# alipay/PainlessInferenceAcceleration

Hardware: NVIDIA H100
Metric: accepted tokens/sec @ Llama-2-7B 64-draft/8-branch; mean accepted len/step (higher is better)
Workload: dtype bf16

## Files before the change

painlessinferenceacceleration_b200/csrc/gemm_ws.cu:

```cuda
#include <cuda.h>
#include <cuda_bf16.h>

#include <new>

#include "common.cuh"

namespace pia {
namespace gemm {

constexpr int BMW = 128;
constexpr int BK = 64;
constexpr int TOK = 64;
constexpr int NTHREADS = 288;
constexpr int PRODUCER_WARP = 8;
constexpr int W_BYTES = BMW * BK * 2, X_BYTES = TOK * BK * 2, STAGE_BYTES = W_BYTES + X_BYTES;
constexpr int XCH_BYTES = TOK * 64 * 2;
constexpr int smem_total(int nstage) { return nstage * STAGE_BYTES + 256 + XCH_BYTES + 1024; }
constexpr int ACC_OFF = 32 * 1024, ACC_LD = TOK + 4;
static_assert(ACC_OFF + BMW * ACC_LD * 4 <= 4 * STAGE_BYTES, "accumulator staging must fit in the pipeline stages");

__device__ __forceinline__ uint32_t smem_u32(const void *p) { return (uint32_t)__cvta_generic_to_shared(p); }
__device__ __forceinline__ void mbar_init(uint32_t bar, int count) {
  asm volatile("mbarrier.init.shared::cta.b64 [%0], %1;" ::"r"(bar), "r"(count));
}
__device__ __forceinline__ void mbar_arrive(uint32_t bar) {
  asm volatile("mbarrier.arrive.shared::cta.b64 _, [%0];" ::"r"(bar) : "memory");
}
__device__ __forceinline__ void mbar_expect_tx(uint32_t bar, uint32_t bytes) {
  asm volatile("mbarrier.arrive.expect_tx.shared::cta.b64 _, [%0], %1;" ::"r"(bar), "r"(bytes) : "memory");
}
__device__ __forceinline__ void mbar_wait(uint32_t bar, uint32_t parity) {
  uint32_t done;
  do {
    asm volatile(
        "{\n\t.reg .pred p;\n\t"
        "mbarrier.try_wait.parity.shared::cta.b64 p, [%1], %2;\n\t"
        "selp.u32 %0, 1, 0, p;\n\t}"
        : "=r"(done)
        : "r"(bar), "r"(parity)
        : "memory");
  } while (!done);
}
__device__ __forceinline__ void cluster_sync_all() {
  asm volatile("barrier.cluster.arrive.release.aligned;\n\tbarrier.cluster.wait.acquire.aligned;" ::: "memory");
}
__device__ __forceinline__ uint32_t map_to_cta(uint32_t local_smem_addr, uint32_t cta_rank) {
  uint32_t r;
  asm volatile("mapa.shared::cluster.u32 %0, %1, %2;" : "=r"(r) : "r"(local_smem_addr), "r"(cta_rank));
  return r;
}
__device__ __forceinline__ void st_cluster_f4(uint32_t addr, float a, float b, float c, float d) {
  asm volatile("st.shared::cluster.v4.f32 [%0], {%1, %2, %3, %4};" ::"r"(addr), "f"(a), "f"(b), "f"(c), "f"(d) : "memory");
}
__device__ __forceinline__ void tma_load_2d(uint32_t dst, const CUtensorMap *map, uint32_t bar, int c0, int c1) {
  asm volatile(
      "cp.async.bulk.tensor.2d.shared::cluster.global.mbarrier::complete_tx::bytes [%0], [%1, {%3, %4}], [%2];"
      ::"r"(dst), "l"(map), "r"(bar), "r"(c0), "r"(c1)
      : "memory");
}
__device__ __forceinline__ void tma_load_3d(uint32_t dst, const CUtensorMap *map, uint32_t bar, int c0, int c1, int c2) {
  asm volatile(
      "cp.async.bulk.tensor.3d.shared::cluster.global.mbarrier::complete_tx::bytes [%0], [%1, {%3, %4, %5}], [%2];"
      ::"r"(dst), "l"(map), "r"(bar), "r"(c0), "r"(c1), "r"(c2)
      : "memory");
}
__device__ __forceinline__ uint64_t kmajor_desc(uint32_t saddr) {
  uint64_t d = 0;
  d |= (uint64_t)((saddr >> 4) & 0x3FFF);
  d |= (uint64_t)1 << 16;
  d |= (uint64_t)(1024 >> 4) << 32;
  d |= (uint64_t)1 << 62;
  return d;
}
__device__ __forceinline__ void wgmma_fence() { asm volatile("wgmma.fence.sync.aligned;" ::: "memory"); }
__device__ __forceinline__ void wgmma_commit() { asm volatile("wgmma.commit_group.sync.aligned;" ::: "memory"); }
__device__ __forceinline__ void wgmma_wait_all() { asm volatile("wgmma.wait_group.sync.aligned 0;" ::: "memory"); }
__device__ __forceinline__ void fence_acc(float (&d)[32]) {
#pragma unroll
  for (int i = 0; i < 32; ++i) asm volatile("" : "+f"(d[i])::"memory");
}
__device__ __forceinline__ void wgmma_m64n64k16(float (&d)[32], uint64_t desc_a, uint64_t desc_b) {
  asm volatile(
      "{\n\t"
      "wgmma.mma_async.sync.aligned.m64n64k16.f32.bf16.bf16 "
      "{%0, %1, %2, %3, %4, %5, %6, %7, %8, %9, %10, %11, %12, %13, %14, %15, "
      "%16, %17, %18, %19, %20, %21, %22, %23, %24, %25, %26, %27, %28, %29, %30, %31}, %32, %33, 1, 1, 1, 0, 0;\n\t}"
      : "+f"(d[0]), "+f"(d[1]), "+f"(d[2]), "+f"(d[3]), "+f"(d[4]), "+f"(d[5]), "+f"(d[6]), "+f"(d[7]), "+f"(d[8]),
        "+f"(d[9]), "+f"(d[10]), "+f"(d[11]), "+f"(d[12]), "+f"(d[13]), "+f"(d[14]), "+f"(d[15]), "+f"(d[16]),
        "+f"(d[17]), "+f"(d[18]), "+f"(d[19]), "+f"(d[20]), "+f"(d[21]), "+f"(d[22]), "+f"(d[23]), "+f"(d[24]),
        "+f"(d[25]), "+f"(d[26]), "+f"(d[27]), "+f"(d[28]), "+f"(d[29]), "+f"(d[30]), "+f"(d[31])
      : "l"(desc_a), "l"(desc_b)
      : "memory");
}
__device__ __forceinline__ void mma_stage(float (&acc)[32], uint32_t wa, uint32_t xa) {
  wgmma_fence();
#pragma unroll
  for (int j = 0; j < BK / 16; ++j) wgmma_m64n64k16(acc, kmajor_desc(wa + j * 32), kmajor_desc(xa + j * 32));
  wgmma_commit();
  wgmma_wait_all();
  fence_acc(acc);
}
__device__ __forceinline__ int frag_row(int warp, int lane, int h) { return 16 * (warp & 3) + (lane >> 2) + 8 * h; }
__device__ __forceinline__ int frag_tok(int lane, int i) { return 8 * i + 2 * (lane & 3); }

struct Params {
  int N, K, n_split, chunks_per_split, n_chunks, rows, tiled;
  int groups, w_group_rows, x_group_chunks;
  long long out_group_stride;
  int cluster;
  int silu;
  int no_pdl;
  __nv_bfloat16 *out_bf16;
  float *out_f32;
};

template <int NSTAGE>
__global__ void __launch_bounds__(NTHREADS, NSTAGE <= 4 ? 2 : 1)
k_gemm_ws(const __grid_constant__ CUtensorMap map_w, const __grid_constant__ CUtensorMap map_x, Params p) {
  constexpr int SMEM_BAR = NSTAGE * STAGE_BYTES;
  extern __shared__ uint8_t smem_raw[];
  const uint32_t base = (smem_u32(smem_raw) + 1023u) & ~1023u;
  uint8_t *sm = smem_raw + (base - smem_u32(smem_raw));
  const int tid = threadIdx.x, warp = tid >> 5, lane = tid & 31;
  const uint32_t bar_full = base + SMEM_BAR, bar_empty = bar_full + 8 * NSTAGE;
  const int tile = p.cluster ? blockIdx.y : blockIdx.x, split = p.cluster ? blockIdx.x : blockIdx.y;
  const int n0 = tile * BMW;
  const int grp = blockIdx.z;
  const int xk0 = grp * p.x_group_chunks;
  const int c0 = split * p.chunks_per_split;
  int c1 = c0 + p.chunks_per_split;
  if (c1 > p.n_chunks) c1 = p.n_chunks;
  const int nch = c1 - c0;

  if (tid == 0) {
    for (int s = 0; s < NSTAGE; ++s) { mbar_init(bar_full + 8 * s, 1); mbar_init(bar_empty + 8 * s, 8); }
    asm volatile("fence.mbarrier_init.release.cluster;" ::: "memory");
  }
  __syncwarp();
  if (!p.no_pdl) pdl_launch_dependents();
  __syncthreads();

  if (warp == PRODUCER_WARP) {
    if (lane == 0) {
      auto load_w = [&](int i, int s) {
        const uint32_t wd = base + s * STAGE_BYTES;
        if (p.tiled) tma_load_3d(wd, &map_w, bar_full + 8 * s, 0, 0, tile * p.n_chunks + c0 + i);
        else tma_load_2d(wd, &map_w, bar_full + 8 * s, (c0 + i) * BK, grp * p.w_group_rows + n0);
      };
      const int pre = nch < NSTAGE ? nch : NSTAGE;
      for (int i = 0; i < pre; ++i) {
        mbar_expect_tx(bar_full + 8 * i, STAGE_BYTES);
        load_w(i, i);
      }
      pdl_wait();
      for (int i = 0; i < pre; ++i) tma_load_2d(base + i * STAGE_BYTES + W_BYTES, &map_x, bar_full + 8 * i, (xk0 + c0 + i) * BK, 0);
      for (int i = pre; i < nch; ++i) {
        const int s = i % NSTAGE, ph = (i / NSTAGE) & 1;
        mbar_wait(bar_empty + 8 * s, ph ^ 1);
        mbar_expect_tx(bar_full + 8 * s, STAGE_BYTES);
        load_w(i, s);
        tma_load_2d(base + s * STAGE_BYTES + W_BYTES, &map_x, bar_full + 8 * s, (xk0 + c0 + i) * BK, 0);
      }
    }
    __syncwarp();
    if (p.cluster) { cluster_sync_all(); cluster_sync_all(); }
    return;
  }

  pdl_wait();
  const int wg = warp >> 2;
  float acc[32];
#pragma unroll
  for (int j = 0; j < 32; ++j) acc[j] = 0.f;
  for (int i = 0; i < nch; ++i) {
    const int s = i % NSTAGE, ph = (i / NSTAGE) & 1;
    mbar_wait(bar_full + 8 * s, ph);
    const uint32_t wa = base + s * STAGE_BYTES, xa = wa + W_BYTES;
    mma_stage(acc, wa + wg * 64 * 128, xa);
    __syncwarp();
    if (lane == 0) mbar_arrive(bar_empty + 8 * s);
  }
  float *accs = reinterpret_cast<float *>(sm + ACC_OFF);
  asm volatile("bar.sync 2, 256;" ::: "memory");
#pragma unroll
  for (int h = 0; h < 2; ++h) {
    const int r = wg * 64 + frag_row(warp, lane, h);
#pragma unroll
    for (int i = 0; i < 8; ++i)
      *reinterpret_cast<float2 *>(accs + r * ACC_LD + frag_tok(lane, i)) = make_float2(acc[4 * i + 2 * h], acc[4 * i + 2 * h + 1]);
  }
  asm volatile("bar.sync 2, 256;" ::: "memory");
  if (wg == 1) {
    if (p.cluster) { cluster_sync_all(); cluster_sync_all(); }
    return;
  }

  const int q = warp;
  const int n = n0 + q * 32 + lane;
  uint32_t v[64];
  {
    const float4 *src = reinterpret_cast<const float4 *>(accs + (q * 32 + lane) * ACC_LD);
#pragma unroll
    for (int t = 0; t < 16; ++t) {
      const float4 a = src[t];
      v[4 * t] = __float_as_uint(a.x); v[4 * t + 1] = __float_as_uint(a.y);
      v[4 * t + 2] = __float_as_uint(a.z); v[4 * t + 3] = __float_as_uint(a.w);
    }
  }
  if (p.cluster) {
    const int cs = p.cluster, RS = BMW / cs;
    cluster_sync_all();
    {
      const int row = q * 32 + lane;
      const int owner = row / RS, rl = row % RS;
      const uint32_t dst = map_to_cta(base + (uint32_t)((split * 16) * RS + rl) * 16, owner);
#pragma unroll
      for (int tq = 0; tq < 16; ++tq)
        st_cluster_f4(dst + (uint32_t)(tq * RS) * 16, __uint_as_float(v[4 * tq]), __uint_as_float(v[4 * tq + 1]),
                      __uint_as_float(v[4 * tq + 2]), __uint_as_float(v[4 * tq + 3]));
    }
    cluster_sync_all();
    {
      const int e = warp * 32 + lane;
      const int rl = e % RS, tg = e / RS;
      const int qpt = RS / 8;
      const int n_out = n0 + split * RS + rl;
      const float4 *buf = reinterpret_cast<const float4 *>(sm);
      __nv_bfloat16 *ob = p.out_bf16 + grp * p.out_group_stride;
      if (n_out < p.N) {
        for (int tq = tg * qpt; tq < (tg + 1) * qpt; ++tq) {
          float4 a = buf[(0 * 16 + tq) * RS + rl];
          for (int src = 1; src < cs; ++src) {
            const float4 b = buf[(src * 16 + tq) * RS + rl];
            a.x += b.x; a.y += b.y; a.z += b.z; a.w += b.w;
          }
          const int t0 = 4 * tq;
          if (t0 < p.rows) ob[(long long)t0 * p.N + n_out] = __float2bfloat16_rn(a.x);
          if (t0 + 1 < p.rows) ob[(long long)(t0 + 1) * p.N + n_out] = __float2bfloat16_rn(a.y);
          if (t0 + 2 < p.rows) ob[(long long)(t0 + 2) * p.N + n_out] = __float2bfloat16_rn(a.z);
          if (t0 + 3 < p.rows) ob[(long long)(t0 + 3) * p.N + n_out] = __float2bfloat16_rn(a.w);
        }
      }
    }
  } else
  if (p.silu) {
    __nv_bfloat16 *xu = reinterpret_cast<__nv_bfloat16 *>(sm + SMEM_BAR + 256);
    __nv_bfloat16 *xg = xu + 32 * 64;
    const int rr = (q & 1) * 32 + lane;
    if (q >= 2) {
#pragma unroll
      for (int t = 0; t < 32; ++t) xu[t * 64 + rr] = __float2bfloat16_rn(__uint_as_float(v[t]));
    } else {
#pragma unroll
      for (int t = 0; t < 32; ++t) xg[t * 64 + rr] = __float2bfloat16_rn(__uint_as_float(v[32 + t]));
    }
    asm volatile("bar.sync 1, 128;" ::: "memory");
    const int col = tile * 64 + rr;
    const int inter = p.N >> 1;
    if (col < inter) {
      const int tb = q < 2 ? 0 : 32;
#pragma unroll
      for (int t = 0; t < 32; ++t) {
        if (tb + t < p.rows) {
          const float g = q < 2 ? __bfloat162float(__float2bfloat16_rn(__uint_as_float(v[t]))) : __bfloat162float(xg[t * 64 + rr]);
          const float u = q < 2 ? __bfloat162float(xu[t * 64 + rr]) : __bfloat162float(__float2bfloat16_rn(__uint_as_float(v[32 + t])));
          const float sg = __bfloat162float(__float2bfloat16_rn(g / (1.f + expf(-g))));
          p.out_bf16[(long long)(tb + t) * inter + col] = __float2bfloat16_rn(sg * u);
        }
      }
    }
  } else
  if (n < p.N) {
    if (p.n_split == 1) {
#pragma unroll
      for (int t = 0; t < TOK; ++t)
        if (t < p.rows) p.out_bf16[grp * p.out_group_stride + (long long)t * p.N + n] = __float2bfloat16_rn(__uint_as_float(v[t]));
    } else {
      float *o = p.out_f32 + (long long)split * TOK * p.N;
#pragma unroll
      for (int t = 0; t < TOK; ++t)
        if (t < p.rows) o[(long long)t * p.N + n] = __uint_as_float(v[t]);
    }
  }
}


struct SkParams {
  int N, n_tiles, n_chunks, rows, max_contrib;
  long long units;
  __nv_bfloat16 *out;
  float *ws;
  int *flags;
};

__device__ __forceinline__ long long sk_begin(long long b, long long U, int G) { return b * U / G; }
__device__ __forceinline__ int sk_cta_of(long long x, long long U, int G) {
  int b = (int)(x * G / U);
  while (b + 1 < G && sk_begin(b + 1, U, G) <= x) ++b;
  while (b > 0 && sk_begin(b, U, G) > x) --b;
  return b;
}

constexpr int SK_STAGES = 8;
constexpr int SK_SMEM_BAR = SK_STAGES * STAGE_BYTES;
constexpr int SK_SMEM_TOTAL = SK_SMEM_BAR + 256 + 1024;

__global__ void __launch_bounds__(NTHREADS, 1)
k_gemm_sk(const __grid_constant__ CUtensorMap map_w, const __grid_constant__ CUtensorMap map_x, SkParams p) {
  extern __shared__ uint8_t smem_raw[];
  const uint32_t base = (smem_u32(smem_raw) + 1023u) & ~1023u;
  const int tid = threadIdx.x, warp = tid >> 5, lane = tid & 31;
  const uint32_t bar_full = base + SK_SMEM_BAR, bar_empty = bar_full + 8 * SK_STAGES;
  const int G = gridDim.x, b = blockIdx.x;
  const long long u0 = sk_begin(b, p.units, G), u1 = sk_begin(b + 1, p.units, G);

  if (tid == 0) {
    for (int s = 0; s < SK_STAGES; ++s) { mbar_init(bar_full + 8 * s, 1); mbar_init(bar_empty + 8 * s, 8); }
    asm volatile("fence.mbarrier_init.release.cluster;" ::: "memory");
  }
  __syncwarp();
  pdl_launch_dependents();
  __syncthreads();
  pdl_wait();

  if (warp == PRODUCER_WARP) {
    if (lane == 0) {
      int i = 0;
      for (long long u = u0; u < u1; ++u, ++i) {
        const int tile = (int)(u / p.n_chunks), ch = (int)(u % p.n_chunks);
        const int s = i % SK_STAGES, ph = (i / SK_STAGES) & 1;
        mbar_wait(bar_empty + 8 * s, ph ^ 1);
        mbar_expect_tx(bar_full + 8 * s, STAGE_BYTES);
        const uint32_t wd = base + s * STAGE_BYTES, xd = wd + W_BYTES;
        tma_load_3d(wd, &map_w, bar_full + 8 * s, 0, 0, tile * p.n_chunks + ch);
        tma_load_2d(xd, &map_x, bar_full + 8 * s, ch * BK, 0);
      }
    }
    return;
  }

  const int wg = warp >> 2;
  int i = 0;
  long long u = u0;
  float acc[32];
  while (u < u1) {
    const int tile = (int)(u / p.n_chunks);
    const long long ts = (long long)tile * p.n_chunks;
    long long ue = ts + p.n_chunks;
    if (ue > u1) ue = u1;
    const bool head = (u == ts), whole = head && (ue == ts + p.n_chunks);
#pragma unroll
    for (int j = 0; j < 32; ++j) acc[j] = 0.f;
    for (; u < ue; ++u, ++i) {
      const int s = i % SK_STAGES, ph = (i / SK_STAGES) & 1;
      mbar_wait(bar_full + 8 * s, ph);
      const uint32_t wa = base + s * STAGE_BYTES, xa = wa + W_BYTES;
      mma_stage(acc, wa + wg * 64 * 128, xa);
      __syncwarp();
      if (lane == 0) mbar_arrive(bar_empty + 8 * s);
    }
    if (!head) {
      const int owner = sk_cta_of(ts, p.units, G);
      const int slot = b - owner - 1;
      float *ws = p.ws + ((long long)tile * p.max_contrib + slot) * BMW * TOK;
#pragma unroll
      for (int h = 0; h < 2; ++h) {
        const int r = wg * 64 + frag_row(warp, lane, h);
#pragma unroll
        for (int k = 0; k < 8; ++k)
          *reinterpret_cast<float2 *>(ws + r * TOK + frag_tok(lane, k)) = make_float2(acc[4 * k + 2 * h], acc[4 * k + 2 * h + 1]);
      }
      __threadfence();
      asm volatile("bar.sync 1, 256;" ::: "memory");
      if (tid == 0) atomicAdd(&p.flags[tile], 1);
    } else {
      if (!whole) {
        const int last = sk_cta_of(ts + p.n_chunks - 1, p.units, G);
        const int contributors = last - b;
        if (tid == 0) {
          while (atomicAdd(&p.flags[tile], 0) < contributors) __nanosleep(64);
          p.flags[tile] = 0;
        }
        asm volatile("bar.sync 1, 256;" ::: "memory");
        __threadfence();
        for (int c = 0; c < contributors; ++c) {
          const float *ws = p.ws + ((long long)tile * p.max_contrib + c) * BMW * TOK;
#pragma unroll
          for (int h = 0; h < 2; ++h) {
            const int r = wg * 64 + frag_row(warp, lane, h);
#pragma unroll
            for (int k = 0; k < 8; ++k) {
              const float2 x = __ldcg(reinterpret_cast<const float2 *>(ws + r * TOK + frag_tok(lane, k)));
              acc[4 * k + 2 * h] += x.x;
              acc[4 * k + 2 * h + 1] += x.y;
            }
          }
        }
      }
#pragma unroll
      for (int h = 0; h < 2; ++h) {
        const int n = tile * BMW + wg * 64 + frag_row(warp, lane, h);
        if (n < p.N) {
#pragma unroll
          for (int k = 0; k < 8; ++k) {
            const int t = frag_tok(lane, k);
            if (t < p.rows) p.out[(long long)t * p.N + n] = __float2bfloat16_rn(acc[4 * k + 2 * h]);
            if (t + 1 < p.rows) p.out[(long long)(t + 1) * p.N + n] = __float2bfloat16_rn(acc[4 * k + 2 * h + 1]);
          }
        }
      }
    }
  }
}

}
}

using namespace pia;
using namespace pia::gemm;

struct pia_gemm_plan {
  CUtensorMap map_w, map_x;
  Params p;
  int nstage;
  int no_pdl;
  int stream_k, sk_grid;
  SkParams sk;
};

typedef CUresult (*EncodeTiledFn)(CUtensorMap *, CUtensorMapDataType, cuuint32_t, void *, const cuuint64_t *,
                                  const cuuint64_t *, const cuuint32_t *, const cuuint32_t *, CUtensorMapInterleave,
                                  CUtensorMapSwizzle, CUtensorMapL2promotion, CUtensorMapFloatOOBfill);

static EncodeTiledFn get_encode() {
  static EncodeTiledFn fn = nullptr;
  if (!fn) {
    cudaDriverEntryPointQueryResult qres;
    void *ptr = nullptr;
    if (cudaGetDriverEntryPoint("cuTensorMapEncodeTiled", &ptr, cudaEnableDefault, &qres) == cudaSuccess &&
        qres == cudaDriverEntryPointSuccess) fn = (EncodeTiledFn)ptr;
  }
  return fn;
}

static int encode_tiled_w(CUtensorMap *m, const void *base, uint64_t n_blocks) {
  EncodeTiledFn fn = get_encode();
  PIA_REQUIRE(fn, "cuTensorMapEncodeTiled not available in this driver");
  cuuint64_t dims[3] = {(cuuint64_t)BK, (cuuint64_t)BMW, n_blocks};
  cuuint64_t strides[2] = {(cuuint64_t)BK * 2, (cuuint64_t)BK * BMW * 2};
  cuuint32_t box[3] = {BK, BMW, 1};
  cuuint32_t estr[3] = {1, 1, 1};
  CUresult r = fn(m, CU_TENSOR_MAP_DATA_TYPE_BFLOAT16, 3, const_cast<void *>(base), dims, strides, box, estr,
                  CU_TENSOR_MAP_INTERLEAVE_NONE, CU_TENSOR_MAP_SWIZZLE_128B, CU_TENSOR_MAP_L2_PROMOTION_L2_256B,
                  CU_TENSOR_MAP_FLOAT_OOB_FILL_NONE);
  if (r != CUDA_SUCCESS) { set_error("cuTensorMapEncodeTiled failed with CUresult %d", (int)r); return PIA_ERR_CUDA; }
  return PIA_OK;
}

static int encode_2d(CUtensorMap *m, const void *base, uint64_t inner, uint64_t outer, uint32_t box_inner,
                     uint32_t box_outer, CUtensorMapL2promotion promo) {
  static EncodeTiledFn fn = nullptr;
  if (!fn) {
    cudaDriverEntryPointQueryResult qres;
    void *ptr = nullptr;
    PIA_CUDA_CHECK(cudaGetDriverEntryPoint("cuTensorMapEncodeTiled", &ptr, cudaEnableDefault, &qres));
    PIA_REQUIRE(ptr && qres == cudaDriverEntryPointSuccess, "cuTensorMapEncodeTiled not available in this driver");
    fn = (EncodeTiledFn)ptr;
  }
  cuuint64_t dims[2] = {inner, outer};
  cuuint64_t strides[1] = {inner * 2};
  cuuint32_t box[2] = {box_inner, box_outer};
  cuuint32_t estr[2] = {1, 1};
  CUresult r = fn(m, CU_TENSOR_MAP_DATA_TYPE_BFLOAT16, 2, const_cast<void *>(base), dims, strides, box, estr,
                  CU_TENSOR_MAP_INTERLEAVE_NONE, CU_TENSOR_MAP_SWIZZLE_128B, promo, CU_TENSOR_MAP_FLOAT_OOB_FILL_NONE);
  if (r != CUDA_SUCCESS) { set_error("cuTensorMapEncodeTiled failed with CUresult %d", (int)r); return PIA_ERR_CUDA; }
  return PIA_OK;
}

extern "C" int pia_gemm_plan_create(const void *d_w, int N, int K, const void *d_x, int x_rows, int split_k,
                                    int w_tiled, pia_gemm_plan_t **out) {
  PIA_REQUIRE(d_w && d_x && out, "null argument");
  PIA_REQUIRE(N > 0 && K > 0 && K % BK == 0, "K must be a multiple of %d", BK);
  PIA_REQUIRE(x_rows >= TOK, "the activation buffer must hold at least %d rows", TOK);
  PIA_REQUIRE((reinterpret_cast<uintptr_t>(d_w) & 15) == 0 && (reinterpret_cast<uintptr_t>(d_x) & 15) == 0, "operands must be 16-byte aligned");
  pia_gemm_plan *g = new (std::nothrow) pia_gemm_plan();
  PIA_REQUIRE(g, "out of host memory");
  const int n_chunks = K / BK;
  const int want_stream_k = (split_k == -1);
  const int want_cluster = (split_k == -2 || split_k == -4 || split_k == -8) ? -split_k : 0;
  if (split_k < -1 && !want_cluster) { delete g; set_error("cluster split-K supports 2, 4 or 8 CTAs"); return PIA_ERR_INVALID; }
  if (want_cluster) split_k = want_cluster;
  if (split_k < 1) split_k = 1;
  if (split_k > n_chunks) split_k = n_chunks;
  g->p.N = N; g->p.K = K; g->p.n_chunks = n_chunks;
  g->p.chunks_per_split = (n_chunks + split_k - 1) / split_k;
  g->p.n_split = (n_chunks + g->p.chunks_per_split - 1) / g->p.chunks_per_split;
  g->p.rows = TOK; g->p.out_bf16 = nullptr; g->p.out_f32 = nullptr; g->p.silu = 0;
  g->p.groups = 1; g->p.w_group_rows = 0; g->p.x_group_chunks = 0; g->p.out_group_stride = 0;
  g->p.cluster = 0;
  if (want_cluster) {
    if (g->p.n_split != want_cluster) { delete g; set_error("K = %d is too short for %d cluster splits", K, want_cluster); return PIA_ERR_INVALID; }
    g->p.cluster = want_cluster;
  }
  g->p.tiled = w_tiled ? 1 : 0;
  if (w_tiled && N % BMW != 0) { delete g; set_error("a tiled weight needs N %% %d == 0", BMW); return PIA_ERR_INVALID; }
  int rc = w_tiled ? encode_tiled_w(&g->map_w, d_w, (uint64_t)(N / BMW) * n_chunks)
                   : encode_2d(&g->map_w, d_w, (uint64_t)K, (uint64_t)N, BK, BMW, CU_TENSOR_MAP_L2_PROMOTION_L2_256B);
  if (rc == PIA_OK) rc = encode_2d(&g->map_x, d_x, (uint64_t)K, (uint64_t)x_rows, BK, TOK, CU_TENSOR_MAP_L2_PROMOTION_L2_256B);
  if (rc == PIA_OK) {
    int n_sm = 132, dev = 0;
    cudaGetDevice(&dev);
    cudaDeviceGetAttribute(&n_sm, cudaDevAttrMultiProcessorCount, dev);
    const int ctas = ((N + BMW - 1) / BMW) * g->p.n_split;
    g->nstage = ctas <= n_sm ? 8 : 4;
    cudaError_t e = cudaFuncSetAttribute(k_gemm_ws<4>, cudaFuncAttributeMaxDynamicSharedMemorySize, smem_total(4));
    if (e == cudaSuccess) e = cudaFuncSetAttribute(k_gemm_ws<8>, cudaFuncAttributeMaxDynamicSharedMemorySize, smem_total(8));
    if (e != cudaSuccess) { set_error("cudaFuncSetAttribute: %s", cudaGetErrorString(e)); rc = PIA_ERR_CUDA; }
  }
  g->stream_k = 0; g->no_pdl = 0;
  if (rc == PIA_OK && want_stream_k) {
    if (!w_tiled) { delete g; set_error("stream-K needs the tiled weight layout"); return PIA_ERR_INVALID; }
    int n_sm = 132, dev = 0;
    cudaGetDevice(&dev);
    cudaDeviceGetAttribute(&n_sm, cudaDevAttrMultiProcessorCount, dev);
    SkParams &k = g->sk;
    k.N = N; k.n_tiles = N / BMW; k.n_chunks = n_chunks; k.rows = TOK;
    k.units = (long long)k.n_tiles * n_chunks;
    g->sk_grid = (int)(k.units < n_sm ? k.units : n_sm);
    const long long per = (k.units + g->sk_grid - 1) / g->sk_grid;
    k.max_contrib = (int)((n_chunks + per - 1) / per) + 1;
    k.out = nullptr;
    cudaError_t e = cudaMalloc((void **)&k.ws, sizeof(float) * (size_t)k.n_tiles * k.max_contrib * BMW * TOK);
    if (e == cudaSuccess) e = cudaMalloc((void **)&k.flags, sizeof(int) * k.n_tiles);
    if (e == cudaSuccess) e = cudaMemset(k.flags, 0, sizeof(int) * k.n_tiles);
    if (e == cudaSuccess) e = cudaFuncSetAttribute(k_gemm_sk, cudaFuncAttributeMaxDynamicSharedMemorySize, SK_SMEM_TOTAL);
    if (e == cudaSuccess) e = cudaDeviceSynchronize();
    if (e != cudaSuccess) { set_error("stream-K plan: %s", cudaGetErrorString(e)); delete g; return PIA_ERR_CUDA; }
    g->stream_k = 1;
    g->p.n_split = 1;
  }
  if (rc != PIA_OK) { delete g; return rc; }
  *out = g;
  return PIA_OK;
}

extern "C" int pia_gemm_plan_destroy(pia_gemm_plan_t *g) {
  if (g) {
    if (g->stream_k) { cudaFree(g->sk.ws); cudaFree(g->sk.flags); }
    delete g;
  }
  return PIA_OK;
}
extern "C" int pia_gemm_plan_set_pdl(pia_gemm_plan_t *g, int on) {
  PIA_REQUIRE(g, "null plan");
  g->no_pdl = on ? 0 : 1;
  return PIA_OK;
}
extern "C" int pia_gemm_plan_splits(const pia_gemm_plan_t *g) { return g ? (g->p.cluster ? 1 : g->p.n_split) : 0; }
extern "C" int pia_gemm_plan_set_silu(pia_gemm_plan_t *g, int on) {
  PIA_REQUIRE(g && g->p.n_split == 1 && !g->stream_k && g->p.N % BMW == 0, "the SiLU*up epilogue needs split_k == 1 and N %% 128 == 0");
  g->p.silu = on ? 1 : 0;
  return PIA_OK;
}

extern "C" int pia_gemm_plan_create_grouped(const void *d_w, int groups, int N, int K, const void *d_x, int x_rows,
                                            pia_gemm_plan_t **out) {
  PIA_REQUIRE(d_w && d_x && out, "null argument");
  PIA_REQUIRE(groups >= 1 && groups <= 65535 && N > 0 && N % BMW == 0 && K > 0 && K % BK == 0,
              "grouped GEMM needs N %% %d == 0 and K %% %d == 0", BMW, BK);
  PIA_REQUIRE(x_rows >= TOK, "the activation buffer must hold at least %d rows", TOK);
  PIA_REQUIRE((reinterpret_cast<uintptr_t>(d_w) & 15) == 0 && (reinterpret_cast<uintptr_t>(d_x) & 15) == 0, "operands must be 16-byte aligned");
  pia_gemm_plan *g = new (std::nothrow) pia_gemm_plan();
  PIA_REQUIRE(g, "out of host memory");
  const int n_chunks = K / BK;
  g->p.N = N; g->p.K = K; g->p.n_chunks = n_chunks; g->p.chunks_per_split = n_chunks; g->p.n_split = 1;
  g->p.rows = TOK; g->p.out_bf16 = nullptr; g->p.out_f32 = nullptr; g->p.silu = 0; g->p.tiled = 0; g->p.cluster = 0;
  g->p.groups = groups; g->p.w_group_rows = N; g->p.x_group_chunks = n_chunks; g->p.out_group_stride = (long long)TOK * N;
  g->stream_k = 0; g->no_pdl = 0;
  int rc = encode_2d(&g->map_w, d_w, (uint64_t)K, (uint64_t)groups * N, BK, BMW, CU_TENSOR_MAP_L2_PROMOTION_L2_256B);
  if (rc == PIA_OK) rc = encode_2d(&g->map_x, d_x, (uint64_t)groups * K, (uint64_t)x_rows, BK, TOK, CU_TENSOR_MAP_L2_PROMOTION_L2_256B);
  if (rc == PIA_OK) {
    int n_sm = 132, dev = 0;
    cudaGetDevice(&dev);
    cudaDeviceGetAttribute(&n_sm, cudaDevAttrMultiProcessorCount, dev);
    g->nstage = (N / BMW) * groups <= n_sm ? 8 : 4;
    cudaError_t e = cudaFuncSetAttribute(k_gemm_ws<4>, cudaFuncAttributeMaxDynamicSharedMemorySize, smem_total(4));
    if (e == cudaSuccess) e = cudaFuncSetAttribute(k_gemm_ws<8>, cudaFuncAttributeMaxDynamicSharedMemorySize, smem_total(8));
    if (e != cudaSuccess) { set_error("cudaFuncSetAttribute: %s", cudaGetErrorString(e)); rc = PIA_ERR_CUDA; }
  }
  if (rc != PIA_OK) { delete g; return rc; }
  *out = g;
  return PIA_OK;
}

struct PdlScope { int on; explicit PdlScope(int off) : on(off) { if (on) ++pia::g_pdl_off; } ~PdlScope() { if (on) --pia::g_pdl_off; } };

extern "C" int pia_gemm_run(pia_gemm_plan_t *g, int rows, void *d_out, void *stream) {
  PIA_REQUIRE(g && d_out, "null argument");
  PIA_REQUIRE(rows >= 1 && rows <= TOK, "rows %d outside [1,%d]", rows, TOK);
  PdlScope pdl_scope(g->no_pdl);
  if (g->stream_k) {
    SkParams k = g->sk;
    k.rows = rows;
    k.out = (__nv_bfloat16 *)d_out;
    PIA_CUDA_CHECK(launch_kernel(k_gemm_sk, dim3(g->sk_grid), dim3(NTHREADS), SK_SMEM_TOTAL, (cudaStream_t)stream, g->map_w, g->map_x, k));
    count_launch();
    return PIA_OK;
  }
  Params p = g->p;
  p.rows = rows; p.no_pdl = g->no_pdl;
  if (p.n_split == 1 || p.cluster) p.out_bf16 = (__nv_bfloat16 *)d_out; else p.out_f32 = (float *)d_out;
  if (p.cluster) {
    dim3 cgrid(p.n_split, (p.N + BMW - 1) / BMW);
    if (g->nstage == 8) PIA_CUDA_CHECK(launch_kernel_cluster(k_gemm_ws<8>, cgrid, dim3(NTHREADS), smem_total(8), (cudaStream_t)stream, (unsigned)p.cluster, g->map_w, g->map_x, p));
    else PIA_CUDA_CHECK(launch_kernel_cluster(k_gemm_ws<4>, cgrid, dim3(NTHREADS), smem_total(4), (cudaStream_t)stream, (unsigned)p.cluster, g->map_w, g->map_x, p));
    count_launch();
    return PIA_OK;
  }
  dim3 grid((p.N + BMW - 1) / BMW, p.n_split, p.groups);
  if (g->nstage == 8) PIA_CUDA_CHECK(launch_kernel(k_gemm_ws<8>, grid, dim3(NTHREADS), smem_total(8), (cudaStream_t)stream, g->map_w, g->map_x, p));
  else PIA_CUDA_CHECK(launch_kernel(k_gemm_ws<4>, grid, dim3(NTHREADS), smem_total(4), (cudaStream_t)stream, g->map_w, g->map_x, p));
  count_launch();
  return PIA_OK;
}
```

painlessinferenceacceleration_b200/models/llama/modeling_llama.py:

```python
import glob
import json
import os

import torch
from torch import nn

from ...common import ops
from ...common.pretrained_model import LookaheadPreTrainedModel


class LlamaRMSNorm(nn.Module):
    def __init__(self, hidden_size, eps=1e-6, device=None, dtype=None):
        super().__init__()
        self.weight = nn.Parameter(torch.ones(hidden_size, device=device, dtype=dtype))
        self.variance_epsilon = eps


class LlamaAttention(nn.Module):
    def __init__(self, cfg, device, dtype):
        super().__init__()
        hd = cfg.hidden_size // cfg.num_attention_heads
        kv = getattr(cfg, 'num_key_value_heads', None) or cfg.num_attention_heads
        kw = dict(bias=False, device=device, dtype=dtype)
        self.q_proj = nn.Linear(cfg.hidden_size, cfg.num_attention_heads * hd, **kw)
        self.k_proj = nn.Linear(cfg.hidden_size, kv * hd, **kw)
        self.v_proj = nn.Linear(cfg.hidden_size, kv * hd, **kw)
        self.o_proj = nn.Linear(cfg.num_attention_heads * hd, cfg.hidden_size, **kw)


class LlamaMLP(nn.Module):
    def __init__(self, cfg, device, dtype):
        super().__init__()
        kw = dict(bias=False, device=device, dtype=dtype)
        self.gate_proj = nn.Linear(cfg.hidden_size, cfg.intermediate_size, **kw)
        self.up_proj = nn.Linear(cfg.hidden_size, cfg.intermediate_size, **kw)
        self.down_proj = nn.Linear(cfg.intermediate_size, cfg.hidden_size, **kw)


class LlamaDecoderLayer(nn.Module):
    def __init__(self, cfg, device, dtype):
        super().__init__()
        self.self_attn = LlamaAttention(cfg, device, dtype)
        self.mlp = self._make_mlp(cfg, device, dtype)
        self.input_layernorm = LlamaRMSNorm(cfg.hidden_size, cfg.rms_norm_eps, device, dtype)
        self.post_attention_layernorm = LlamaRMSNorm(cfg.hidden_size, cfg.rms_norm_eps, device, dtype)

    def _make_mlp(self, cfg, device, dtype):
        return LlamaMLP(cfg, device, dtype)


class LlamaModel(nn.Module):
    layer_cls = LlamaDecoderLayer

    def __init__(self, cfg, device, dtype):
        super().__init__()
        self.embed_tokens = nn.Embedding(cfg.vocab_size, cfg.hidden_size, device=device, dtype=dtype)
        self.layers = nn.ModuleList([self.layer_cls(cfg, device, dtype) for _ in range(cfg.num_hidden_layers)])
        self.norm = LlamaRMSNorm(cfg.hidden_size, cfg.rms_norm_eps, device, dtype)


class LlamaForCausalLM(LookaheadPreTrainedModel):
    model_cls = LlamaModel

    def __init__(self, config, device=None, dtype=torch.bfloat16):
        super().__init__(config)
        if device is None:
            device = torch.device('cuda', torch.cuda.current_device()) if torch.cuda.is_available() else 'meta'
        assert dtype == torch.bfloat16, 'the H100 path computes in bf16'
        self.model = self.model_cls(config, device, dtype)
        self.lm_head = nn.Linear(config.hidden_size, config.vocab_size, bias=False, device=device, dtype=dtype)
        self._fused = False
        for p_ in self.parameters():
            p_.requires_grad_(False)

    @torch.no_grad()
    def init_weights(self, seed=0, std=0.02):
        gen = torch.Generator(device=self.device)
        gen.manual_seed(seed)
        for name, p in self.named_parameters():
            if name.endswith('layernorm.weight') or name.endswith('norm.weight'):
                p.fill_(1.0)
            else:
                p.normal_(0.0, std, generator=gen)
        return self

    @classmethod
    def from_pretrained(cls, path, torch_dtype=torch.bfloat16, device=None, **kwargs):
        from transformers import AutoConfig
        config = AutoConfig.from_pretrained(path)
        model = cls(config, device=device, dtype=torch_dtype)
        files = sorted(glob.glob(os.path.join(path, '*.safetensors')))
        own = dict(model.named_parameters())
        seen = set()
        if files:
            from safetensors.torch import load_file
            shards = (load_file(f) for f in files)
        else:
            shards = (torch.load(f, map_location='cpu') for f in sorted(glob.glob(os.path.join(path, 'pytorch_model*.bin'))))
        with torch.no_grad():
            for sd in shards:
                for k, v in model._convert_checkpoint_keys(sd).items():
                    if k in own:
                        own[k].copy_(v.to(torch_dtype))
                        seen.add(k)
        if 'lm_head.weight' not in seen and getattr(config, 'tie_word_embeddings', False):
            with torch.no_grad():
                model.lm_head.weight.copy_(model.model.embed_tokens.weight)
            seen.add('lm_head.weight')
        missing = [k for k in own if k not in seen]
        if missing:
            raise RuntimeError(f'checkpoint is missing {len(missing)} tensors, e.g. {missing[:4]}')
        return model

    def _convert_checkpoint_keys(self, sd):
        return sd

    def fuse(self):
        if self._fused:
            return
        for layer in self.model.layers:
            a = layer.self_attn
            w = torch.cat([a.q_proj.weight.data, a.k_proj.weight.data, a.v_proj.weight.data], dim=0).contiguous()
            nq, nk = a.q_proj.weight.shape[0], a.k_proj.weight.shape[0]
            a.q_proj.weight.data, a.k_proj.weight.data, a.v_proj.weight.data = w[:nq], w[nq:nq + nk], w[nq + nk:]
            a.qkv_weight = w
            self._fuse_mlp(layer)
        self._fused = True

    def _fuse_mlp(self, layer):
        m = layer.mlp
        w = torch.cat([m.gate_proj.weight.data, m.up_proj.weight.data], dim=0).contiguous()
        ni = m.gate_proj.weight.shape[0]
        m.gate_proj.weight.data, m.up_proj.weight.data = w[:ni], w[ni:]
        m.gate_up_weight = w

    def geometry(self):
        c = self.config
        hd = c.hidden_size // c.num_attention_heads
        return dict(n_layers=c.num_hidden_layers, hidden=c.hidden_size, n_q_heads=c.num_attention_heads,
                    n_kv_heads=getattr(c, 'num_key_value_heads', None) or c.num_attention_heads, head_dim=hd,
                    inter=c.intermediate_size, vocab=c.vocab_size)

    def rope_tables(self, max_pos):
        c = self.config
        hd = c.hidden_size // c.num_attention_heads
        rp = getattr(c, 'rope_parameters', None) or {}
        theta = float(getattr(c, 'rope_theta', None) or rp.get('rope_theta', 10000.0))
        scaling = getattr(c, 'rope_scaling', None) or ({k: v for k, v in rp.items() if k != 'rope_theta'} if rp else None)
        rtype = (scaling or {}).get('rope_type', (scaling or {}).get('type', 'default')) if scaling else 'default'
        dev = self.device
        inv_freq = 1.0 / (theta ** (torch.arange(0, hd, 2, dtype=torch.int64).float().to(dev) / hd))
        pos = torch.arange(max_pos, device=dev).float()
        if rtype in (None, 'default'):
            pass
        elif rtype == 'linear':
            pos = pos / float(scaling['factor'])
        elif rtype == 'dynamic':
            factor, mpe = float(scaling['factor']), int(c.max_position_embeddings)
            if max_pos > mpe:
                base = theta * ((factor * max_pos / mpe) - (factor - 1)) ** (hd / (hd - 2))
                inv_freq = 1.0 / (base ** (torch.arange(0, hd, 2, dtype=torch.int64).float().to(dev) / hd))
        else:
            raise ValueError(f'Unknown RoPE scaling type {rtype}')
        freqs = pos[:, None] * inv_freq[None, :]
        return freqs.cos().to(torch.bfloat16).contiguous(), freqs.sin().to(torch.bfloat16).contiguous()

    def _gemm_plans(self, rt):
        plans = getattr(rt, 'gemm_plans', None)
        if plans is not None:
            return plans
        import os
        if os.environ.get('PIA_GEMM', '1') == '0' or rt.max_nodes != 64:
            rt.gemm_plans = False
            return False
        b = rt.decode_bufs
        g = rt.g
        dev = b.y.device
        b.gu = torch.zeros((b.rows, 2 * g['inter']), dtype=torch.bfloat16, device=dev)
        b.act = torch.zeros((b.rows, g['inter']), dtype=torch.bfloat16, device=dev)
        plans = {'layers': []}
        for layer in self.model.layers:
            plans['layers'].append(self._layer_gemm_plans(layer, b))
        plans['lm_head'] = self._mk_gemm(self.lm_head.weight.data, b.y)
        rt.gemm_plans = plans
        return plans

    def _layer_gemm_plans(self, layer, b):
        import os
        want = os.environ.get('PIA_GEMM_SET', 'gate_up').split(',')
        plans = {}
        if 'gate_up_silu' in want and layer.mlp.gate_up_weight.shape[0] % 256 == 0:
            cache = self.__dict__.setdefault('_tiled_weights', {})
            key = ('gate_up_silu', layer.mlp.gate_up_weight.data_ptr())
            if key not in cache:
                cache[key] = ops.tile_weight(ops.interleave_gate_up(layer.mlp.gate_up_weight))
            plans['gate_up_silu'] = ops.Gemm(cache[key], b.y, tiled=True).set_silu()
        elif 'gate_up' in want or 'gate_up_silu' in want:
            plans['gate_up'] = self._mk_gemm(layer.mlp.gate_up_weight, b.y)
        if 'qkv' in want:
            plans['qkv'] = self._mk_gemm(layer.self_attn.qkv_weight, b.y)
        sk = int(os.environ.get('PIA_GEMM_SPLIT', '-4'))
        if 'qkv2' in want:
            plans['qkv'] = self._mk_gemm(layer.self_attn.qkv_weight, b.y, split_k=-2)
        if 'o' in want:
            plans['o'] = self._mk_gemm(layer.self_attn.o_proj.weight.data, b.attn, split_k=sk)
        if 'down' in want and layer.mlp.down_proj.weight.shape[1] % 64 == 0 and layer.mlp.down_proj.weight.shape[1] >= 64 * abs(sk):
            plans['down'] = self._mk_gemm(layer.mlp.down_proj.weight.data, b.act, split_k=sk)
        for name in os.environ.get('PIA_GEMM_NOPDL', '').split(','):
            if name in plans:
                plans[name].set_pdl(False)
        return plans

    def _mk_gemm(self, w, x, split_k=1):
        if w.shape[0] % 128 == 0:
            cache = self.__dict__.setdefault('_tiled_weights', {})
            key = (w.data_ptr(), tuple(w.shape))
            if key not in cache:
                cache[key] = ops.tile_weight(w)
            return ops.Gemm(cache[key], x, split_k=split_k, tiled=True)
        return ops.Gemm(w.contiguous(), x, split_k=split_k)

    def _prefetch_cfg(self, rt):
        cfg = getattr(rt, 'prefetch_cfg', None)
        if cfg is None:
            import os
            spec = os.environ.get('PIA_PREFETCH', '0')
            v = [float(t) for t in spec.split(',')] if spec not in ('', '0') else []
            cfg = False
            if v and torch.cuda.is_available():
                v = (v + [0.0] * 4)[:4]
                cfg = dict(o=v[0], gate_up=v[1], down=v[2], rate=v[3], side=torch.cuda.Stream(device=self.device))
            rt.prefetch_cfg = cfg
        return cfg

    @staticmethod
    def _prefetch(pf, jobs):
        main = torch.cuda.current_stream()
        pf['side'].wait_stream(main)
        with torch.cuda.stream(pf['side']):
            for (t, frac, tile_bytes) in jobs:
                if frac <= 0:
                    continue
                total = t.numel() * t.element_size()
                if tile_bytes:
                    rb = max(16384, int(tile_bytes * min(frac, 1.0)) // 16384 * 16384)
                    ops.l2_prefetch(t, n_ranges=total // tile_bytes, stride_bytes=tile_bytes, range_bytes=min(rb, tile_bytes),
                                    gbytes_per_s=pf['rate'])
                else:
                    ops.l2_prefetch(t, range_bytes=int(total * min(frac, 1.0)) // 16 * 16, gbytes_per_s=pf['rate'])
        pf['dirty'] = True

    def _mlp(self, rt, layer, y, plans=None, pf=None):
        m = layer.mlp
        if plans:
            b = rt.decode_bufs
            if 'gate_up_silu' in plans:
                plans['gate_up_silu'].run(64, out=b.act)
            else:
                if 'gate_up' in plans:
                    plans['gate_up'].run(64, out=b.gu)
                else:
                    torch.mm(y, m.gate_up_weight.t(), out=b.gu)
                if pf:
                    self._prefetch(pf, [(m.down_proj.weight, pf['down'], 0)])
                ops.silu_mul(b.gu, b.act)
            if 'down' in plans:
                o = plans['down'].run(64)
                return (o, None) if plans['down'].splits == 1 else (None, o)
            return torch.mm(b.act, m.down_proj.weight.t()), None
        gu = torch.mm(y, m.gate_up_weight.t())
        act = torch.empty((gu.shape[0], gu.shape[1] // 2), dtype=gu.dtype, device=gu.device)
        ops.silu_mul(gu, act)
        return torch.mm(act, m.down_proj.weight.t()), None

    def _verify_layers(self, rt, bufs=None, last_only=False):
        self.fuse()
        b = bufs if bufs is not None else rt.decode_bufs
        g = rt.g
        eps = self.config.rms_norm_eps
        ops.embed_gather(self.model.embed_tokens.weight, b.ids, b.n_total, b.h)
        plans = self._gemm_plans(rt) if b is rt.decode_bufs else False
        pf = self._prefetch_cfg(rt) if plans else False
        fused_attn = b is rt.decode_bufs and os.environ.get('PIA_ATTN_FUSED', '0') != '0' and \
            (b.slots.batch == 1 or b.slots.kv_slot_stride != 0)
        x, parts, resid_in = b.h, None, None

        def norm(w):
            if parts is not None:
                ops.rmsnorm_partials(parts, resid_in, w, eps, b.resid, b.y)
            else:
                ops.rmsnorm(x, resid_in, w, eps, b.resid, b.y)

        for li, layer in enumerate(self.model.layers):
            lp = plans['layers'][li] if plans else None
            norm(layer.input_layernorm.weight)
            a = layer.self_attn
            if lp and 'qkv' in lp:
                lp['qkv'].run(64, out=b.qkv)
            else:
                torch.mm(b.y, a.qkv_weight.t(), out=b.qkv)
            if pf and lp and 'gate_up' in lp:
                gw = lp['gate_up'].weight
                self._prefetch(pf, [(a.o_proj.weight, pf['o'], 0),
                                    (gw, pf['gate_up'], gw.shape[1] * gw.shape[2] * gw.shape[3] * 2 if gw.dim() == 4 else 0)])
            if fused_attn:
                rt.plan.forward_fused(li, b.qkv, b.mask, b.slots, rt.rope_cos, rt.rope_sin, b.attn)
            else:
                ops.rope_kv_append(b.qkv, b.mask, b.slots, g['n_q_heads'], g['n_kv_heads'], g['head_dim'], rt.rope_cos,
                                   rt.rope_sin, b.q, rt.k_layer(li, b.kv_slot), rt.v_layer(li, b.kv_slot), rt.max_seq)
                rt.plan.forward(li, b.q, b.mask, b.slots, b.attn)
            if lp and 'o' in lp:
                o = lp['o'].run(64)
                x, parts, resid_in = (o, None, b.resid) if lp['o'].splits == 1 else (None, o, b.resid)
            else:
                x, parts, resid_in = torch.mm(b.attn, a.o_proj.weight.t()), None, b.resid
            norm(layer.post_attention_layernorm.weight)
            x, parts = self._mlp(rt, layer, b.y, lp, pf)
        if pf and pf.pop('dirty', False):
            torch.cuda.current_stream().wait_stream(pf['side'])
        if last_only:
            return
        norm(self.model.norm.weight)
        if b.logits is not None:
            if plans:
                plans['lm_head'].run(64, out=b.logits)
            else:
                torch.mm(b.y, self.lm_head.weight.t(), out=b.logits)


class LlamaPreTrainedModel(LookaheadPreTrainedModel):
    pass
```

painlessinferenceacceleration_b200/models/mixtral/modeling_mixtral.py:

```python
import torch
from torch import nn

from ...common import ops
from ..llama.modeling_llama import LlamaDecoderLayer, LlamaForCausalLM, LlamaModel
from ..mistral.modeling_mistral import warn_sliding_window


class MixtralRouter(nn.Module):
    def __init__(self, cfg, device, dtype):
        super().__init__()
        self.weight = nn.Parameter(torch.empty((cfg.num_local_experts, cfg.hidden_size), device=device, dtype=dtype))


class MixtralExperts(nn.Module):
    def __init__(self, cfg, device, dtype):
        super().__init__()
        E, H, I = cfg.num_local_experts, cfg.hidden_size, cfg.intermediate_size
        self.gate_up_proj = nn.Parameter(torch.empty((E, 2 * I, H), device=device, dtype=dtype))
        self.down_proj = nn.Parameter(torch.empty((E, H, I), device=device, dtype=dtype))


class MixtralSparseMoeBlock(nn.Module):
    def __init__(self, cfg, device, dtype):
        super().__init__()
        self.top_k = cfg.num_experts_per_tok
        self.num_experts = cfg.num_local_experts
        self.gate = MixtralRouter(cfg, device, dtype)
        self.experts = MixtralExperts(cfg, device, dtype)


class MixtralDecoderLayer(LlamaDecoderLayer):
    def _make_mlp(self, cfg, device, dtype):
        return MixtralSparseMoeBlock(cfg, device, dtype)


class MixtralModel(LlamaModel):
    layer_cls = MixtralDecoderLayer


class MixtralForCausalLM(LlamaForCausalLM):
    model_cls = MixtralModel

    def _fuse_mlp(self, layer):
        pass

    def rope_tables(self, max_pos):
        warn_sliding_window(self.config, max_pos)
        return super().rope_tables(max_pos)

    def _convert_checkpoint_keys(self, sd):
        import re
        out = {}
        pend = self.__dict__.setdefault('_pending_experts', {})
        E = self.config.num_local_experts
        pat = re.compile(r'^(model\.layers\.\d+)\.block_sparse_moe\.experts\.(\d+)\.(w1|w2|w3)\.weight$')
        for k, v in sd.items():
            m = pat.match(k)
            if m:
                pend.setdefault(m.group(1), {})[(int(m.group(2)), m.group(3))] = v
            elif '.block_sparse_moe.gate.weight' in k:
                out[k.replace('.block_sparse_moe.gate.weight', '.mlp.gate.weight')] = v
            else:
                out[k] = v
        for layer in list(pend):
            parts = pend[layer]
            if len(parts) == 3 * E:
                out[layer + '.mlp.experts.gate_up_proj'] = torch.stack(
                    [torch.cat([parts[(e, 'w1')], parts[(e, 'w3')]], dim=0) for e in range(E)], dim=0)
                out[layer + '.mlp.experts.down_proj'] = torch.stack([parts[(e, 'w2')] for e in range(E)], dim=0)
                del pend[layer]
        return out

    def geometry(self):
        g = super().geometry()
        g['n_experts'] = self.config.num_local_experts
        return g

    def _layer_gemm_plans(self, layer, b):
        import os
        moe = layer.mlp
        E, two_i, H = moe.experts.gate_up_proj.shape
        inter = two_i // 2
        if os.environ.get('PIA_MOE_GEMM', '1') == '0' or H % 128 or H % 64 or inter % 64 or (E * two_i) % 128:
            return {}
        dev = b.y.device
        if not hasattr(b, 'moe_gu'):
            b.moe_gu = torch.zeros((b.rows, E * two_i), dtype=torch.bfloat16, device=dev)
            b.moe_act = torch.zeros((b.rows, E * inter), dtype=torch.bfloat16, device=dev)
            b.moe_out = torch.zeros((b.rows, H), dtype=torch.bfloat16, device=dev)
            b.moe_dense = torch.zeros((b.rows, E), dtype=torch.bfloat16, device=dev)
        return {'moe_gate_up': ops.Gemm(moe.experts.gate_up_proj.data.view(E * two_i, H), b.y),
                'moe_down': ops.Gemm.grouped(moe.experts.down_proj.data, b.moe_act)}

    def _mlp(self, rt, layer, y, plans=None, pf=None):
        moe = layer.mlp
        if plans:
            b = rt.decode_bufs
            E = moe.num_experts
            inter = moe.experts.down_proj.shape[2]
            ops.moe_router(y, moe.gate.weight, moe.top_k, b.moe_dense)
            plans['moe_gate_up'].run(64, out=b.moe_gu)
            ops.silu_mul(b.moe_gu.view(b.rows * E, 2 * inter), b.moe_act.view(b.rows * E, inter))
            ye = plans['moe_down'].run(64)
            ops.moe_combine(ye, b.moe_dense, b.moe_out)
            return b.moe_out, None
        dense = torch.empty((y.shape[0], moe.num_experts), dtype=y.dtype, device=y.device)
        ops.moe_router(y, moe.gate.weight, moe.top_k, dense)
        out = torch.zeros_like(y)
        inter = moe.experts.down_proj.shape[2]
        act = torch.empty((y.shape[0], inter), dtype=y.dtype, device=y.device)
        for e in range(moe.num_experts):
            gu = torch.mm(y, moe.experts.gate_up_proj[e].t())
            ops.silu_mul(gu, act)
            ye = torch.mm(act, moe.experts.down_proj[e].t())
            out += ye * dense[:, e:e + 1]
        return out, None
```

Baseline: 535.9.

## Swizzle GEMM accumulator staging and default to fused gate_up+SiLU plan

The GEMM epilogue drops the padded accumulator row stride and uses an XOR swizzle on 16-byte chunks, so the fragment writes and float4 row reads avoid shared-memory bank conflicts without padding. On the Python side, the env-driven GEMM plan selection (qkv, o, down, split-K partials, PDL toggles) is removed. Each layer now always uses the fused gate_up+SiLU tiled GEMM when the shape allows, and falls back to torch.mm for qkv, o and down. This changes the default from a plain gate_up GEMM plus a separate silu_mul to the fused variant, and removes the optional split-K paths.

```diff
diff --git a/painlessinferenceacceleration_b200/csrc/gemm_ws.cu b/painlessinferenceacceleration_b200/csrc/gemm_ws.cu
--- a/painlessinferenceacceleration_b200/csrc/gemm_ws.cu
+++ b/painlessinferenceacceleration_b200/csrc/gemm_ws.cu
@@ -16,8 +16,10 @@
 constexpr int W_BYTES = BMW * BK * 2, X_BYTES = TOK * BK * 2, STAGE_BYTES = W_BYTES + X_BYTES;
 constexpr int XCH_BYTES = TOK * 64 * 2;
 constexpr int smem_total(int nstage) { return nstage * STAGE_BYTES + 256 + XCH_BYTES + 1024; }
-constexpr int ACC_OFF = 32 * 1024, ACC_LD = TOK + 4;
+constexpr int ACC_OFF = 32 * 1024, ACC_LD = TOK;
 static_assert(ACC_OFF + BMW * ACC_LD * 4 <= 4 * STAGE_BYTES, "accumulator staging must fit in the pipeline stages");
+__device__ __forceinline__ int acc_swz(int r) { return ((r & 3) << 1) | ((r >> 2) & 1); }
+__device__ __forceinline__ int acc_idx(int r, int tok) { return r * ACC_LD + (((tok >> 2) ^ acc_swz(r)) << 2) + (tok & 3); }
 
 __device__ __forceinline__ uint32_t smem_u32(const void *p) { return (uint32_t)__cvta_generic_to_shared(p); }
 __device__ __forceinline__ void mbar_init(uint32_t bar, int count) {
@@ -187,7 +189,7 @@
     const int r = wg * 64 + frag_row(warp, lane, h);
 #pragma unroll
     for (int i = 0; i < 8; ++i)
-      *reinterpret_cast<float2 *>(accs + r * ACC_LD + frag_tok(lane, i)) = make_float2(acc[4 * i + 2 * h], acc[4 * i + 2 * h + 1]);
+      *reinterpret_cast<float2 *>(accs + acc_idx(r, frag_tok(lane, i))) = make_float2(acc[4 * i + 2 * h], acc[4 * i + 2 * h + 1]);
   }
   asm volatile("bar.sync 2, 256;" ::: "memory");
   if (wg == 1) {
@@ -199,10 +201,11 @@
   const int n = n0 + q * 32 + lane;
   uint32_t v[64];
   {
-    const float4 *src = reinterpret_cast<const float4 *>(accs + (q * 32 + lane) * ACC_LD);
+    const int r = q * 32 + lane, swz = acc_swz(r);
+    const float4 *src = reinterpret_cast<const float4 *>(accs + r * ACC_LD);
 #pragma unroll
     for (int t = 0; t < 16; ++t) {
-      const float4 a = src[t];
+      const float4 a = src[t ^ swz];
       v[4 * t] = __float_as_uint(a.x); v[4 * t + 1] = __float_as_uint(a.y);
       v[4 * t + 2] = __float_as_uint(a.z); v[4 * t + 3] = __float_as_uint(a.w);
     }
diff --git a/painlessinferenceacceleration_b200/models/llama/modeling_llama.py b/painlessinferenceacceleration_b200/models/llama/modeling_llama.py
--- a/painlessinferenceacceleration_b200/models/llama/modeling_llama.py
+++ b/painlessinferenceacceleration_b200/models/llama/modeling_llama.py
@@ -186,39 +186,25 @@
         return plans
 
     def _layer_gemm_plans(self, layer, b):
-        import os
-        want = os.environ.get('PIA_GEMM_SET', 'gate_up').split(',')
-        plans = {}
-        if 'gate_up_silu' in want and layer.mlp.gate_up_weight.shape[0] % 256 == 0:
-            cache = self.__dict__.setdefault('_tiled_weights', {})
-            key = ('gate_up_silu', layer.mlp.gate_up_weight.data_ptr())
-            if key not in cache:
-                cache[key] = ops.tile_weight(ops.interleave_gate_up(layer.mlp.gate_up_weight))
-            plans['gate_up_silu'] = ops.Gemm(cache[key], b.y, tiled=True).set_silu()
-        elif 'gate_up' in want or 'gate_up_silu' in want:
-            plans['gate_up'] = self._mk_gemm(layer.mlp.gate_up_weight, b.y)
-        if 'qkv' in want:
-            plans['qkv'] = self._mk_gemm(layer.self_attn.qkv_weight, b.y)
-        sk = int(os.environ.get('PIA_GEMM_SPLIT', '-4'))
-        if 'qkv2' in want:
-            plans['qkv'] = self._mk_gemm(layer.self_attn.qkv_weight, b.y, split_k=-2)
-        if 'o' in want:
-            plans['o'] = self._mk_gemm(layer.self_attn.o_proj.weight.data, b.attn, split_k=sk)
-        if 'down' in want and layer.mlp.down_proj.weight.shape[1] % 64 == 0 and layer.mlp.down_proj.weight.shape[1] >= 64 * abs(sk):
-            plans['down'] = self._mk_gemm(layer.mlp.down_proj.weight.data, b.act, split_k=sk)
-        for name in os.environ.get('PIA_GEMM_NOPDL', '').split(','):
-            if name in plans:
-                plans[name].set_pdl(False)
-        return plans
-
-    def _mk_gemm(self, w, x, split_k=1):
+        m = layer.mlp
+        if m.gate_up_weight.shape[1] % 64:
+            return {}
+        if m.gate_up_weight.shape[0] % 256:
+            return {'gate_up': self._mk_gemm(m.gate_up_weight, b.y)}
+        cache = self.__dict__.setdefault('_tiled_weights', {})
+        key = ('gate_up_silu', m.gate_up_weight.data_ptr())
+        if key not in cache:
+            cache[key] = ops.tile_weight(ops.interleave_gate_up(m.gate_up_weight))
+        return {'gate_up_silu': ops.Gemm(cache[key], b.y, tiled=True).set_silu()}
+
+    def _mk_gemm(self, w, x):
         if w.shape[0] % 128 == 0:
             cache = self.__dict__.setdefault('_tiled_weights', {})
             key = (w.data_ptr(), tuple(w.shape))
             if key not in cache:
                 cache[key] = ops.tile_weight(w)
-            return ops.Gemm(cache[key], x, split_k=split_k, tiled=True)
-        return ops.Gemm(w.contiguous(), x, split_k=split_k)
+            return ops.Gemm(cache[key], x, tiled=True)
+        return ops.Gemm(w.contiguous(), x)
 
     def _prefetch_cfg(self, rt):
         cfg = getattr(rt, 'prefetch_cfg', None)
@@ -264,14 +250,11 @@
                 if pf:
                     self._prefetch(pf, [(m.down_proj.weight, pf['down'], 0)])
                 ops.silu_mul(b.gu, b.act)
-            if 'down' in plans:
-                o = plans['down'].run(64)
-                return (o, None) if plans['down'].splits == 1 else (None, o)
-            return torch.mm(b.act, m.down_proj.weight.t()), None
+            return torch.mm(b.act, m.down_proj.weight.t())
         gu = torch.mm(y, m.gate_up_weight.t())
         act = torch.empty((gu.shape[0], gu.shape[1] // 2), dtype=gu.dtype, device=gu.device)
         ops.silu_mul(gu, act)
-        return torch.mm(act, m.down_proj.weight.t()), None
+        return torch.mm(act, m.down_proj.weight.t())
 
     def _verify_layers(self, rt, bufs=None, last_only=False):
         self.fuse()
@@ -283,22 +266,16 @@
         pf = self._prefetch_cfg(rt) if plans else False
         fused_attn = b is rt.decode_bufs and os.environ.get('PIA_ATTN_FUSED', '0') != '0' and \
             (b.slots.batch == 1 or b.slots.kv_slot_stride != 0)
-        x, parts, resid_in = b.h, None, None
+        x, resid_in = b.h, None
 
         def norm(w):
-            if parts is not None:
-                ops.rmsnorm_partials(parts, resid_in, w, eps, b.resid, b.y)
-            else:
-                ops.rmsnorm(x, resid_in, w, eps, b.resid, b.y)
+            ops.rmsnorm(x, resid_in, w, eps, b.resid, b.y)
 
         for li, layer in enumerate(self.model.layers):
             lp = plans['layers'][li] if plans else None
             norm(layer.input_layernorm.weight)
             a = layer.self_attn
-            if lp and 'qkv' in lp:
-                lp['qkv'].run(64, out=b.qkv)
-            else:
-                torch.mm(b.y, a.qkv_weight.t(), out=b.qkv)
+            torch.mm(b.y, a.qkv_weight.t(), out=b.qkv)
             if pf and lp and 'gate_up' in lp:
                 gw = lp['gate_up'].weight
                 self._prefetch(pf, [(a.o_proj.weight, pf['o'], 0),
@@ -309,13 +286,9 @@
                 ops.rope_kv_append(b.qkv, b.mask, b.slots, g['n_q_heads'], g['n_kv_heads'], g['head_dim'], rt.rope_cos,
                                    rt.rope_sin, b.q, rt.k_layer(li, b.kv_slot), rt.v_layer(li, b.kv_slot), rt.max_seq)
                 rt.plan.forward(li, b.q, b.mask, b.slots, b.attn)
-            if lp and 'o' in lp:
-                o = lp['o'].run(64)
-                x, parts, resid_in = (o, None, b.resid) if lp['o'].splits == 1 else (None, o, b.resid)
-            else:
-                x, parts, resid_in = torch.mm(b.attn, a.o_proj.weight.t()), None, b.resid
+            x, resid_in = torch.mm(b.attn, a.o_proj.weight.t()), b.resid
             norm(layer.post_attention_layernorm.weight)
-            x, parts = self._mlp(rt, layer, b.y, lp, pf)
+            x = self._mlp(rt, layer, b.y, lp, pf)
         if pf and pf.pop('dirty', False):
             torch.cuda.current_stream().wait_stream(pf['side'])
         if last_only:
diff --git a/painlessinferenceacceleration_b200/models/mixtral/modeling_mixtral.py b/painlessinferenceacceleration_b200/models/mixtral/modeling_mixtral.py
--- a/painlessinferenceacceleration_b200/models/mixtral/modeling_mixtral.py
+++ b/painlessinferenceacceleration_b200/models/mixtral/modeling_mixtral.py
@@ -103,7 +103,7 @@
             ops.silu_mul(b.moe_gu.view(b.rows * E, 2 * inter), b.moe_act.view(b.rows * E, inter))
             ye = plans['moe_down'].run(64)
             ops.moe_combine(ye, b.moe_dense, b.moe_out)
-            return b.moe_out, None
+            return b.moe_out
         dense = torch.empty((y.shape[0], moe.num_experts), dtype=y.dtype, device=y.device)
         ops.moe_router(y, moe.gate.weight, moe.top_k, dense)
         out = torch.zeros_like(y)
@@ -114,4 +114,4 @@
             ops.silu_mul(gu, act)
             ye = torch.mm(act, moe.experts.down_proj[e].t())
             out += ye * dense[:, e:e + 1]
-        return out, None
+        return out
```

After: 545.2 (median of 6 runs). 1.02x the previous value.
